# carlosluis/multiagent_planning

Measured on AMD Instinct MI355X. Metric: agent-QP solves/sec (K=15 horizon), higher is better.
Workload: dtype f64

## Files before the change

multiagent_planning_amd/csrc/dmpc_lists.hip:

```cpp

constexpr int NSEG = 3, SEG_STEPS = K / NSEG;
static_assert(NSEG * SEG_STEPS == K, "horizon segments");
template <typename TT>
__global__ void bbox_kernel(int total, int C, const TT *__restrict__ lT, float *__restrict__ bbox, float *__restrict__ bbox_nm )
{
    const int i = blockIdx.x * blockDim.x + threadIdx.x;
    if (i >= total) return;
    const int c = i % C;
    const size_t gs = (size_t)(i / C);
    const TT *src = lT + gs * N3 * C + c;
    float *dst = bbox + gs * (6 * NSEG) * C + c;
    for (int sg = 0; sg < NSEG; ++sg) {
        double lo[3] = {1e300, 1e300, 1e300}, hi[3] = {-1e300, -1e300, -1e300};
        for (int k = sg * SEG_STEPS; k < (sg + 1) * SEG_STEPS; ++k)
#pragma unroll
            for (int a = 0; a < 3; ++a) {
                const double v = (double)src[(size_t)(3 * k + a) * C];
                lo[a] = fmin(lo[a], v); hi[a] = fmax(hi[a], v);
            }
#pragma unroll
        for (int a = 0; a < 3; ++a) {
            const float flo = __double2float_rd(lo[a]), fhi = __double2float_ru(hi[a]);
            dst[(size_t)(6 * sg + 2 * a) * C] = flo; dst[(size_t)(6 * sg + 2 * a + 1) * C] = fhi;
            bbox_nm[(size_t)i * NBOX_NM + 6 * sg + 2 * a] = flo; bbox_nm[(size_t)i * NBOX_NM + 6 * sg + 2 * a + 1] = fhi;
        }
    }
}

template <typename TT>
__device__ __forceinline__ float nbrmajor_word(const TT *lT, int C, size_t t)
{
    const int l = (int)(t & 63), k4 = l >> 2, a4 = l & 3;
    const size_t gc = t >> 6, gs = gc / (size_t)C, c = gc - gs * (size_t)C;
    return (a4 < 3 && k4 < K) ? (float)lT[(gs * N3 + 3 * k4 + a4) * C + c] : 0.f;
}
template <typename TT>
__global__ void table_nbrmajor_kernel(size_t total, int C, const TT *__restrict__ lT, float *__restrict__ out, int *__restrict__ zbuf , size_t nz)
{
    const size_t t = (size_t)blockIdx.x * blockDim.x + threadIdx.x;
    for (size_t z = t; z < nz; z += (size_t)gridDim.x * blockDim.x) zbuf[z] = 0;
    if (t >= total) return;
    out[t] = nbrmajor_word(lT, C, t);
}

typedef float f4_t __attribute__((ext_vector_type(4)));
typedef const f4_t __attribute__((address_space(4))) *ConstF4;
__global__ __launch_bounds__(64) void nbr_kernel(int S, int G, int C, int g_local, int c_first, int c_count, int short_from, float R, float Rz,
                                                 const float *__restrict__ bbox, const float *__restrict__ bbox_nm, int cap, int *__restrict__ list,
                                                 int *__restrict__ cnt_out)
{
    constexpr int NB = 6 * NSEG;
    const int nblk = (c_count + 63) >> 6;
    const int part = blockIdx.x % NBR_PARTS, sb = blockIdx.x / NBR_PARTS;
    const int scene = sb / nblk, b = sb - scene * nblk;
    const int lane = threadIdx.x;
    const int ci = b * 64 + lane;
    const bool mine = ci < c_count;
    const int cl = c_first + (mine ? ci : 0);
    float ob[NB];
#pragma unroll
    for (int x = 0; x < NB; ++x) {
        const float v = bbox[((size_t)(g_local * S + scene) * NB + x) * C + cl];
        const float infl = (x % 6 < 4) ? R : Rz;
        ob[x] = (x & 1) ? v + infl : v - infl;
    }
    const int pcap = cap / NBR_PARTS;
    const size_t gid = (size_t)scene * c_count + (mine ? ci : 0);
    int *mylist = list + gid * (size_t)cap + (size_t)part * pcap;
    const long E = (long)G * C;
    const int e_lo = (int)(E * part / NBR_PARTS), e_hi = (int)(E * (part + 1) / NBR_PARTS);
    int cnt = 0;
    for (int e = e_lo; e < e_hi;) {
        const int r = e / C, j_lo = e - r * C;
        const int j_hi = (e_hi - e) < (C - j_lo) ? j_lo + (e_hi - e) : C;
        const int j_end = j_hi < C - ((short_from && r >= short_from) ? 1 : 0) ? j_hi : C - ((short_from && r >= short_from) ? 1 : 0);
        const float *base = bbox_nm + ((size_t)(r * S + scene) * C) * NBOX_NM;
        const int self = (r == g_local) ? cl : -1;
        for (int jc = j_lo; jc < j_end; ++jc) {
            const ConstF4 nb = (ConstF4)(unsigned long long)(base + (size_t)jc * NBOX_NM);
            const f4_t n0 = nb[0], n1 = nb[1], n2 = nb[2], n3 = nb[3], n4 = nb[4];
            const float nv[20] = {n0.x, n0.y, n0.z, n0.w, n1.x, n1.y, n1.z, n1.w, n2.x, n2.y, n2.z, n2.w, n3.x, n3.y, n3.z, n3.w, n4.x, n4.y, n4.z, n4.w};
            float sgm[NSEG];
#pragma unroll
            for (int sg = 0; sg < NSEG; ++sg) {
                const float a0 = nv[6 * sg] - ob[6 * sg + 1], a1 = ob[6 * sg] - nv[6 * sg + 1], a2 = nv[6 * sg + 2] - ob[6 * sg + 3];
                const float a3 = ob[6 * sg + 2] - nv[6 * sg + 3], a4 = nv[6 * sg + 4] - ob[6 * sg + 5], a5 = ob[6 * sg + 4] - nv[6 * sg + 5];
                sgm[sg] = fmaxf(__builtin_fmaxf(__builtin_fmaxf(a0, a1), a2), __builtin_fmaxf(__builtin_fmaxf(a3, a4), a5));
            }
            const float worst = __builtin_fminf(__builtin_fminf(sgm[0], sgm[1]), sgm[2]);
            if (worst <= 0.f && mine && jc != self) {
                if (cnt < pcap) mylist[cnt] = (r << 20) | jc;
                cnt++;
            }
        }
        e += j_hi - j_lo;
    }
    if (mine) cnt_out[gid * NBR_PARTS + part] = cnt > pcap ? -1 : cnt;
}

struct GridGeom {
    float org[3], inv[3];
    int n[3];
};
__device__ __forceinline__ int grid_coord(const GridGeom &g, int a, float x)
{
    const float t = (x - g.org[a]) * g.inv[a];
    const int c = (int)floorf(t);
    return c < 0 ? 0 : (c >= g.n[a] ? g.n[a] - 1 : c);
}
__device__ __forceinline__ int box_cell(const GridGeom &gg, const float (&lo)[3], const float (&hi)[3], float (&half)[3])
{
    int cc[3];
#pragma unroll
    for (int a = 0; a < 3; ++a) {
        half[a] = 0.5f * (hi[a] - lo[a]) * 1.0001f + 1e-5f;
        cc[a] = grid_coord(gg, a, 0.5f * (lo[a] + hi[a]));
    }
    return (cc[2] * gg.n[1] + cc[1]) * gg.n[0] + cc[0];
}
__global__ void grid_bin_kernel(int total, int S, int C, int short_from, GridGeom gg, const float *__restrict__ bbox_nm, int *__restrict__ cellof,
                                int *__restrict__ cnt, int *__restrict__ maxhalf)
{
    const int i = blockIdx.x * blockDim.x + threadIdx.x;
    const bool in = i < total;
    const int ii = in ? i : total - 1;
    const int c = ii % C, rs = ii / C, scene = rs % S, r = rs / S;
    const bool valid = in && !(short_from && r >= short_from && c == C - 1);
    const float *b = bbox_nm + (size_t)ii * NBOX_NM;
    const int ncell = gg.n[0] * gg.n[1] * gg.n[2];
    const int sc0 = __builtin_amdgcn_readfirstlane(scene);
    const bool uni = __all(scene == sc0);
    {
        const int sg = (int)blockIdx.y;
        float lo[3], hi[3], half[3];
#pragma unroll
        for (int a = 0; a < 3; ++a) { lo[a] = b[6 * sg + 2 * a]; hi[a] = b[6 * sg + 2 * a + 1]; }
        const int cell = box_cell(gg, lo, hi, half);
#pragma unroll
        for (int a = 0; a < 3; ++a) {
            int hb = valid ? __float_as_int(half[a]) : 0;
            int *dst = maxhalf + ((size_t)scene * NSEG + sg) * 3 + a;
            if (uni) {
#pragma unroll
                for (int off = 32; off > 0; off >>= 1) { const int o = __shfl_xor(hb, off); hb = o > hb ? o : hb; }
                if ((threadIdx.x & 63) == 0 && hb > *(volatile int *)dst) atomicMax(dst, hb);
            } else if (valid && hb > *(volatile int *)dst) atomicMax(dst, hb);
        }
        if (in) cellof[(size_t)sg * total + i] = valid ? cell : -1;
        if (valid) atomicAdd(cnt + ((size_t)scene * NSEG + sg) * ncell + cell, 1);
    }
}
__global__ void grid_scan_kernel(int ncell, int *__restrict__ cnt, int *__restrict__ start)
{
    __shared__ int part[1024];
    int *f = cnt + (size_t)blockIdx.x * ncell, *st = start + (size_t)blockIdx.x * (ncell + 1);
    const int per = (ncell + 1023) / 1024, lo = threadIdx.x * per, hi = lo + per < ncell ? lo + per : ncell;
    int a = 0;
    for (int c = lo; c < hi; ++c) a += f[c];
    part[threadIdx.x] = a;
    __syncthreads();
    for (int d = 1; d < 1024; d <<= 1) {
        const int v = threadIdx.x >= d ? part[threadIdx.x - d] : 0;
        __syncthreads();
        part[threadIdx.x] += v;
        __syncthreads();
    }
    int run = part[threadIdx.x] - a;
    for (int c = lo; c < hi; ++c) { st[c] = run; run += f[c]; f[c] = 0; }
    if (threadIdx.x == 1023) st[ncell] = part[1023];
}
__device__ __forceinline__ void chord_record(const f4_t *row , float e1z, int code, f4_t &r0, f4_t &r1)
{
    f4_t v[SEG_STEPS];
#pragma unroll
    for (int u = 0; u < SEG_STEPS; ++u) { v[u] = row[u]; v[u].z *= e1z; }
    const f4_t a0 = v[0], a1 = v[SEG_STEPS - 1];
    float dev2 = 0.f;
#pragma unroll
    for (int u = 1; u < SEG_STEPS - 1; ++u) {
        const float t = (float)u / (float)(SEG_STEPS - 1);
        const float dx = v[u].x - (a0.x + t * (a1.x - a0.x)), dy = v[u].y - (a0.y + t * (a1.y - a0.y)), dz = v[u].z - (a0.z + t * (a1.z - a0.z));
        dev2 = fmaxf(dev2, dx * dx + dy * dy + dz * dz);
    }
    r0.x = __int_as_float(code); r0.y = a0.x; r0.z = a0.y; r0.w = a0.z;
    r1.x = a1.x - a0.x; r1.y = a1.y - a0.y; r1.z = a1.z - a0.z; r1.w = sqrtf(dev2) * 1.0001f + 1e-5f;
}
__global__ void grid_fill_kernel(int total, int S, int C, int ncell, float e1z, const int *__restrict__ cellof, int *__restrict__ cnt, const int *__restrict__ start,
                                 const float *__restrict__ lrow, f4_t *__restrict__ ent)
{
    const int i = blockIdx.x * blockDim.x + threadIdx.x;
    if (i >= total) return;
    const int c = i % C, rs = i / C, scene = rs % S, r = rs / S;
    const size_t nag = (size_t)total / S;
#pragma unroll
    for (int sg = 0; sg < NSEG; ++sg) {
        const int cell = cellof[(size_t)sg * total + i];
        if (cell < 0) return;
        const size_t ss = (size_t)scene * NSEG + sg;
        const int pos = atomicAdd(cnt + ss * ncell + cell, 1);
        f4_t r0, r1;
        chord_record((const f4_t *)lrow + (size_t)i * 16 + SEG_STEPS * sg, e1z, (r << 20) | c, r0, r1);
        const size_t ei = ss * nag + start[ss * (ncell + 1) + cell] + pos;
        ent[ei] = r0; ent[(size_t)S * NSEG * nag + ei] = r1;
    }
}
template <typename TT>
__global__ __launch_bounds__(256) void grid_prep_kernel(int total, int C, int short_from, GridGeom gg, int nbA, const TT *__restrict__ lT, float *__restrict__ bbox,
                                                        float *__restrict__ bbox_nm, float *__restrict__ lrow, int *__restrict__ cellof, int *__restrict__ posof,
                                                        int *__restrict__ cnt, int *__restrict__ maxhalf)
{
    if ((int)blockIdx.x >= nbA) {
        const size_t t = (size_t)((int)blockIdx.x - nbA) * 256 + threadIdx.x;
        if (t >= (size_t)total * 64) return;
        lrow[t] = nbrmajor_word(lT, C, t);
        return;
    }
    __shared__ int mh[NSEG * 3];
    if (threadIdx.x < NSEG * 3) mh[threadIdx.x] = 0;
    __syncthreads();
    const int i = (int)blockIdx.x * 256 + (int)threadIdx.x;
    if (i < total) {
        const int c = i % C, r = i / C;
        const bool valid = !(short_from && r >= short_from && c == C - 1);
        const TT *src = lT + (size_t)r * N3 * C + c;
        float *dst = bbox + (size_t)r * (6 * NSEG) * C + c;
        const int ncell = gg.n[0] * gg.n[1] * gg.n[2];
#pragma unroll
        for (int sg = 0; sg < NSEG; ++sg) {
            double lo[3] = {1e300, 1e300, 1e300}, hi[3] = {-1e300, -1e300, -1e300};
#pragma unroll
            for (int k = sg * SEG_STEPS; k < (sg + 1) * SEG_STEPS; ++k)
#pragma unroll
                for (int a = 0; a < 3; ++a) {
                    const double v = (double)src[(size_t)(3 * k + a) * C];
                    lo[a] = fmin(lo[a], v); hi[a] = fmax(hi[a], v);
                }
            float flo[3], fhi[3], half[3];
#pragma unroll
            for (int a = 0; a < 3; ++a) {
                flo[a] = __double2float_rd(lo[a]); fhi[a] = __double2float_ru(hi[a]);
                dst[(size_t)(6 * sg + 2 * a) * C] = flo[a]; dst[(size_t)(6 * sg + 2 * a + 1) * C] = fhi[a];
                bbox_nm[(size_t)i * NBOX_NM + 6 * sg + 2 * a] = flo[a]; bbox_nm[(size_t)i * NBOX_NM + 6 * sg + 2 * a + 1] = fhi[a];
            }
            const int cell = box_cell(gg, flo, fhi, half);
#pragma unroll
            for (int a = 0; a < 3; ++a)
                if (valid) atomicMax(&mh[3 * sg + a], __float_as_int(half[a]));
            cellof[(size_t)sg * total + i] = valid ? cell : -1;
            posof[(size_t)sg * total + i] = valid ? atomicAdd(cnt + (size_t)sg * ncell + cell, 1) : 0;
        }
    }
    __syncthreads();
    if (threadIdx.x < NSEG * 3) { const int v = mh[threadIdx.x]; if (v > *(volatile int *)(maxhalf + threadIdx.x)) atomicMax(maxhalf + threadIdx.x, v); }
}
__global__ __launch_bounds__(256) void grid_fill2_kernel(int total, int C, int ncell, float e1z, const int *__restrict__ cellof, const int *__restrict__ posof,
                                                         const int *__restrict__ cnt, int *__restrict__ start, const float *__restrict__ lrow, f4_t *__restrict__ ent)
{
    int *st = (int *)dmpc_smem;
    __shared__ int wtot[NSEG][4];
    const int t = (int)threadIdx.x, lane = t & 63, wave = t >> 6;
    const int chunk = ((ncell + 255) / 256) | 1;
    const int lo = t * chunk, hi = lo + chunk < ncell ? lo + chunk : ncell;
#pragma unroll 4
    for (int j = t; j < ncell; j += 256)
#pragma unroll
        for (int sg = 0; sg < NSEG; ++sg) st[sg * (ncell + 1) + j] = cnt[(size_t)sg * ncell + j];
    __syncthreads();
    int sum[NSEG], inc[NSEG];
#pragma unroll
    for (int sg = 0; sg < NSEG; ++sg) sum[sg] = 0;
    for (int j = lo; j < hi; ++j)
#pragma unroll
        for (int sg = 0; sg < NSEG; ++sg) sum[sg] += st[sg * (ncell + 1) + j];
#pragma unroll
    for (int sg = 0; sg < NSEG; ++sg) inc[sg] = sum[sg];
#pragma unroll
    for (int off = 1; off < 64; off <<= 1)
#pragma unroll
        for (int sg = 0; sg < NSEG; ++sg) { const int o = __shfl_up(inc[sg], off); if (lane >= off) inc[sg] += o; }
    if (lane == 63)
#pragma unroll
        for (int sg = 0; sg < NSEG; ++sg) wtot[sg][wave] = inc[sg];
    __syncthreads();
    int run[NSEG];
#pragma unroll
    for (int sg = 0; sg < NSEG; ++sg) {
        run[sg] = inc[sg] - sum[sg];
        for (int w = 0; w < wave; ++w) run[sg] += wtot[sg][w];
        if (t == 255) st[sg * (ncell + 1) + ncell] = wtot[sg][0] + wtot[sg][1] + wtot[sg][2] + wtot[sg][3];
    }
    for (int j = lo; j < hi; ++j)
#pragma unroll
        for (int sg = 0; sg < NSEG; ++sg) { int *c = st + sg * (ncell + 1) + j; const int n = *c; *c = run[sg]; run[sg] += n; }
    __syncthreads();
    {
        const int all = NSEG * (ncell + 1), slice = (all + (int)gridDim.x - 1) / (int)gridDim.x;
        const int j0 = (int)blockIdx.x * slice, j1 = j0 + slice < all ? j0 + slice : all;
        for (int j = j0 + t; j < j1; j += 256) start[j] = st[j];
    }
    const int i = (int)blockIdx.x * 256 + t;
    if (i >= total) return;
    const int code = ((i / C) << 20) | (i % C);
#pragma unroll
    for (int sg = 0; sg < NSEG; ++sg) {
        const int cell = cellof[(size_t)sg * total + i];
        if (cell < 0) return;
        const int pos = posof[(size_t)sg * total + i];
        f4_t r0, r1;
        chord_record((const f4_t *)lrow + (size_t)i * 16 + SEG_STEPS * sg, e1z, code, r0, r1);
        const size_t ei = (size_t)sg * total + st[sg * (ncell + 1) + cell] + pos;
        ent[ei] = r0; ent[(size_t)NSEG * total + ei] = r1;
    }
}
constexpr int GQ_WAVES = NSEG;
constexpr int GQ_STAGE = 128;
inline size_t grid_query_lds(int nagents, int close_cap = 0)
{
    return (((size_t)((nagents + 31) / 32) * 4 + GQ_WAVES * GQ_STAGE * 4 + 15) & ~(size_t)15) + 16 * 16 + (close_cap > 0 ? 16 + (size_t)close_cap * 8 : 0);
}
typedef float f2_t __attribute__((ext_vector_type(2)));
__global__ __launch_bounds__(64 * GQ_WAVES) void grid_query_kernel(int S, int G, int C, int g_local, int c_first, int c_count, GridGeom gg, float R, float Rz, float e1z, float thr2,
                                                                   const float *__restrict__ bbox_nm, const float *__restrict__ lrow, const int *__restrict__ start,
                                                                   const f4_t *__restrict__ ent, const int *__restrict__ maxhalf, int cap, int cell_order,
                                                                   int *__restrict__ list, int *__restrict__ cnt_out,
                                                                   float thr_close, int close_cap, int *__restrict__ close_list, int *__restrict__ close_cnt)
{
    const int wave = __builtin_amdgcn_readfirstlane((int)(threadIdx.x >> 6)), lane = (int)(threadIdx.x & 63);
    const int gid = (int)blockIdx.x;
    const int nag = G * C, nwords = (nag + 31) >> 5, ncell = gg.n[0] * gg.n[1] * gg.n[2];
    const int scene = gid / c_count;
    int ci = gid - scene * c_count;
    if (cell_order) ci = __builtin_amdgcn_readfirstlane(__float_as_int(ent[(size_t)scene * NSEG * nag + ci].x) & 0xfffff);
    const int cl = c_first + ci;
    const int oid = scene * c_count + ci;
    unsigned *bits = (unsigned *)dmpc_smem;
    int *stage = (int *)(dmpc_smem + (size_t)nwords * 4) + wave * GQ_STAGE;
    f4_t *ownrow = (f4_t *)(dmpc_smem + (((size_t)nwords * 4 + GQ_WAVES * GQ_STAGE * 4 + 15) & ~(size_t)15));
    int *ccnt = (int *)(ownrow + 16), *crec = ccnt + 4;
    for (int i = (int)threadIdx.x; i < nwords; i += 64 * GQ_WAVES) bits[i] = 0u;
    if (close_cap > 0 && threadIdx.x == 0) *ccnt = 0;
    const size_t self_i = (size_t)(g_local * S + scene) * C + cl;
    if (threadIdx.x < 16) ownrow[lane] = ((const f4_t *)lrow)[self_i * 16 + lane];
    const ConstF4 ob4 = (ConstF4)(unsigned long long)(bbox_nm + self_i * NBOX_NM);
    const f4_t o0 = ob4[0], o1 = ob4[1], o2 = ob4[2], o3 = ob4[3], o4 = ob4[4];
    const float obx[18] = {o0.x, o0.y, o0.z, o0.w, o1.x, o1.y, o1.z, o1.w, o2.x, o2.y, o2.z, o2.w, o3.x, o3.y, o3.z, o3.w, o4.x, o4.y};
    __syncthreads();
    const int self_code = (g_local << 20) | cl;
    {
        const int sg = wave;
        int c_lo[3], c_hi[3];
#pragma unroll
        for (int a = 0; a < 3; ++a) {
            const float lo = sg == 0 ? obx[2 * a] : (sg == 1 ? obx[6 + 2 * a] : obx[12 + 2 * a]);
            const float hi = sg == 0 ? obx[2 * a + 1] : (sg == 1 ? obx[6 + 2 * a + 1] : obx[12 + 2 * a + 1]);
            const float infl = a < 2 ? R : Rz;
            const float reach = infl + __int_as_float(maxhalf[((size_t)scene * NSEG + sg) * 3 + a]);
            c_lo[a] = grid_coord(gg, a, lo - reach); c_hi[a] = grid_coord(gg, a, hi + reach);
        }
        f4_t oa0 = ownrow[SEG_STEPS * sg], oa1 = ownrow[SEG_STEPS * sg + SEG_STEPS - 1];
        oa0.z *= e1z; oa1.z *= e1z;
        const float odx = oa1.x - oa0.x, ody = oa1.y - oa0.y, odz = oa1.z - oa0.z;
        float odev2 = 0.f;
#pragma unroll
        for (int u = 1; u < SEG_STEPS - 1; ++u) {
            const f4_t o = ownrow[SEG_STEPS * sg + u];
            const float t = (float)u / (float)(SEG_STEPS - 1);
            const float dx = o.x - (oa0.x + t * odx), dy = o.y - (oa0.y + t * ody), dz = o.z * e1z - (oa0.z + t * odz);
            odev2 = fmaxf(odev2, dx * dx + dy * dy + dz * dz);
        }
        const float lim0 = sqrtf(thr2) + sqrtf(odev2) * 1.0001f + 2e-4f;
        const size_t ss = (size_t)scene * NSEG + sg;
        const int *st = start + ss * (ncell + 1);
        const f4_t *en = ent + ss * nag, *en2 = ent + (size_t)S * NSEG * nag + ss * nag;
        int nst = 0;
        auto traj_test = [&](int n) {
            const bool have = lane < n;
            const int code = stage[have ? lane : 0];
            const int r = code >> 20, jc = code & 0xfffff;
            const f4_t *row = (const f4_t *)lrow + ((size_t)(r * S + scene) * C + jc) * 16 + SEG_STEPS * sg;
            bool pass = false;
            int cmask = 0;
#pragma unroll 1
            for (int u = 0; u < SEG_STEPS; ++u) {
                const f4_t o = ownrow[SEG_STEPS * sg + u], w = row[u];
                const float dx = o.x - w.x, dy = o.y - w.y, dz = (o.z - w.z) * e1z;
                const float d2 = dx * dx + dy * dy + dz * dz;
                pass = pass || (d2 < thr2);
                cmask |= (d2 < thr_close) ? (1 << u) : 0;
            }
            if (have && pass) {
                const int idx = r * C + jc;
                atomicOr(bits + (idx >> 5), 1u << (idx & 31));
                if (cmask != 0) {
                    int pos = atomicAdd(ccnt, __popc(cmask));
                    while (cmask) {
                        const int u = __ffs(cmask) - 1;
                        cmask &= cmask - 1;
                        if (pos < close_cap) { crec[2 * pos] = code; crec[2 * pos + 1] = SEG_STEPS * sg + u; }
                        ++pos;
                    }
                }
            }
        };
        const int ny = c_hi[1] - c_lo[1] + 1, nruns_all = ny * (c_hi[2] - c_lo[2] + 1);
        const UDiv div_ny((unsigned)ny);
        for (int run0 = 0; run0 < nruns_all; run0 += 64) {
            const int nruns = nruns_all - run0 < 64 ? nruns_all - run0 : 64;
            int rb = 0, re = 0;
            if (lane < nruns) {
                int qz, qy;
                div_ny.divmod((unsigned)(run0 + lane), qz, qy);
                const int row0 = ((c_lo[2] + qz) * gg.n[1] + c_lo[1] + qy) * gg.n[0];
                rb = st[row0 + c_lo[0]]; re = st[row0 + c_hi[0] + 1];
            }
            const int len = re - rb;
            int pre = len;
            for (int off = 1; off < 64; off <<= 1) { const int o = __shfl_up(pre, off); if (lane >= off) pre += o; }
            const int tot = __builtin_amdgcn_readlane(pre, 63);
            const int basev = rb - (pre - len);
            const int nround = (tot + 63) >> 6;
            struct Rec { f4_t a, b; bool hv; };
            auto fetch = [&](int k, Rec &rc) {
                const int vi = 64 * k + lane;
                rc.hv = vi < tot;
                const int vq = rc.hv ? vi : tot - 1;
                int j = 0;
#pragma unroll
                for (int step = 32; step > 0; step >>= 1) { const int pm = __shfl(pre, j + step - 1); if (pm <= vq) j += step; }
                const size_t ei = (size_t)(__shfl(basev, j) + vq);
                rc.a = en[ei]; rc.b = en2[ei];
            };
            auto test = [&](const Rec &rc) {
                const float qx = rc.a.y - oa0.x, qy = rc.a.z - oa0.y, qz = rc.a.w - oa0.z;
                const float ex = rc.b.x - odx, ey = rc.b.y - ody, ez = rc.b.z - odz;
                const float ee = ex * ex + ey * ey + ez * ez, qe = qx * ex + qy * ey + qz * ez, qq = qx * qx + qy * qy + qz * qz;
                const float tt = __builtin_fminf(__builtin_fmaxf(-qe * __builtin_amdgcn_rcpf(__builtin_fmaxf(ee, 1e-20f)), 0.f), 1.f);
                const float d2 = qq + tt * (qe + qe + tt * ee);
                const float lim = lim0 + rc.b.w;
                const int c0 = __float_as_int(rc.a.x);
                const bool surv = rc.hv && c0 != self_code && d2 <= lim * lim;
                const unsigned long long m = __ballot(surv);
                if (m) {
                    if (surv) stage[nst + lanes_below(m, lane)] = c0;
                    nst += __popcll(m);
                    LSYNC();
                    if (nst >= 64) {
                        traj_test(64);
                        LSYNC();
                        const int keep = lane < nst - 64 ? stage[64 + lane] : 0;
                        LSYNC();
                        if (lane < nst - 64) stage[lane] = keep;
                        nst -= 64;
                        LSYNC();
                    }
                }
            };
            if (nround > 0) {
                Rec ra, rb2;
                fetch(0, ra);
                for (int k = 0; k < nround; k += 2) {
                    fetch(k + 1 < nround ? k + 1 : nround - 1, rb2);
                    test(ra);
                    if (k + 1 >= nround) break;
                    fetch(k + 2 < nround ? k + 2 : nround - 1, ra);
                    test(rb2);
                }
            }
        }
        if (nst > 0) traj_test(nst);
    }
    __syncthreads();
    if (wave == 1 && close_cap > 0) {
        const int n = *ccnt;
        int *dst = close_list + (size_t)oid * 2 * close_cap;
        if (n <= close_cap) for (int i = lane; i < 2 * n; i += 64) dst[i] = crec[i];
        if (lane == 0) close_cnt[oid] = n > close_cap ? -1 : n;
    }
    if (wave != 0) return;
    int *out = list + (size_t)oid * cap;
    int total = 0;
    const UDiv div_c((unsigned)C);
    for (int w0 = 0; w0 < nwords; w0 += 64) {
        unsigned word = w0 + lane < nwords ? bits[w0 + lane] : 0u;
        const int mycnt = __popc(word);
        int pre = mycnt;
        for (int off = 1; off < 64; off <<= 1) { const int o = __shfl_up(pre, off); if (lane >= off) pre += o; }
        const int wave_total = __builtin_amdgcn_readlane(pre, 63);
        int pos = total + pre - mycnt;
        while (word) {
            const int b = __ffs((int)word) - 1;
            word &= word - 1u;
            const int idx = ((w0 + lane) << 5) + b;
            int r = 0, jc = idx;
            if (G > 1) div_c.divmod((unsigned)idx, r, jc);
            if (pos < cap) out[pos] = (r << 20) | jc;
            ++pos;
        }
        total += wave_total;
    }
    if (lane == 0) cnt_out[(size_t)oid * NBR_PARTS] = total > cap ? -1 : total;
}
```

Baseline: 15.99 million.

## Map candidate slots to grid runs via LDS bitmap windows and DPP scans

Replaces the per-fetch 6-step shuffle binary search, which finds which cell run each candidate slot belongs to, with a per-wave LDS bitmap of run endpoints. Each fetch resolves its run index with mbcnt over that bitmap and reads the run base from LDS. Prefix sums now use DPP row operations instead of shfl_up loops, and the output-compaction loop skips all-zero word groups. The cost is more LDS per wave, extra LDS barriers and atomics for each 2048-slot window, and reliance on specific DPP control encodings being correct for a 64-lane wave.

Result: faster. 16.31 million (median of 6 runs) (+2.0%).

```diff
diff --git a/multiagent_planning_amd/csrc/dmpc_lists.hip b/multiagent_planning_amd/csrc/dmpc_lists.hip
--- a/multiagent_planning_amd/csrc/dmpc_lists.hip
+++ b/multiagent_planning_amd/csrc/dmpc_lists.hip
@@ -314,11 +314,25 @@
 }
 constexpr int GQ_WAVES = NSEG;
 constexpr int GQ_STAGE = 128;
+constexpr int GQ_RUNS = 64;
+constexpr int GQ_WIN = 2048;
+constexpr int GQ_WAVE_INTS = GQ_STAGE + GQ_RUNS + GQ_WIN / 32;
+static_assert(GQ_WIN / 32 == 64, "the window is one word per lane");
 inline size_t grid_query_lds(int nagents, int close_cap = 0)
 {
-    return (((size_t)((nagents + 31) / 32) * 4 + GQ_WAVES * GQ_STAGE * 4 + 15) & ~(size_t)15) + 16 * 16 + (close_cap > 0 ? 16 + (size_t)close_cap * 8 : 0);
+    return (((size_t)((nagents + 31) / 32) * 4 + GQ_WAVES * GQ_WAVE_INTS * 4 + 15) & ~(size_t)15) + 16 * 16 + (close_cap > 0 ? 16 + (size_t)close_cap * 8 : 0);
 }
 typedef float f2_t __attribute__((ext_vector_type(2)));
+__device__ __forceinline__ int wave_scan_add(int v)
+{
+    v += __builtin_amdgcn_update_dpp(0, v, 0x111, 0xf, 0xf, false);
+    v += __builtin_amdgcn_update_dpp(0, v, 0x112, 0xf, 0xf, false);
+    v += __builtin_amdgcn_update_dpp(0, v, 0x114, 0xf, 0xf, false);
+    v += __builtin_amdgcn_update_dpp(0, v, 0x118, 0xf, 0xf, false);
+    v += __builtin_amdgcn_update_dpp(0, v, 0x142, 0xa, 0xf, false);
+    v += __builtin_amdgcn_update_dpp(0, v, 0x143, 0xc, 0xf, false);
+    return v;
+}
 __global__ __launch_bounds__(64 * GQ_WAVES) void grid_query_kernel(int S, int G, int C, int g_local, int c_first, int c_count, GridGeom gg, float R, float Rz, float e1z, float thr2,
                                                                    const float *__restrict__ bbox_nm, const float *__restrict__ lrow, const int *__restrict__ start,
                                                                    const f4_t *__restrict__ ent, const int *__restrict__ maxhalf, int cap, int cell_order,
@@ -334,8 +348,10 @@
     const int cl = c_first + ci;
     const int oid = scene * c_count + ci;
     unsigned *bits = (unsigned *)dmpc_smem;
-    int *stage = (int *)(dmpc_smem + (size_t)nwords * 4) + wave * GQ_STAGE;
-    f4_t *ownrow = (f4_t *)(dmpc_smem + (((size_t)nwords * 4 + GQ_WAVES * GQ_STAGE * 4 + 15) & ~(size_t)15));
+    int *stage = (int *)(dmpc_smem + (size_t)nwords * 4) + wave * GQ_WAVE_INTS;
+    int *runbase = stage + GQ_STAGE;
+    unsigned *win = (unsigned *)(runbase + GQ_RUNS);
+    f4_t *ownrow = (f4_t *)(dmpc_smem + (((size_t)nwords * 4 + GQ_WAVES * GQ_WAVE_INTS * 4 + 15) & ~(size_t)15));
     int *ccnt = (int *)(ownrow + 16), *crec = ccnt + 4;
     for (int i = (int)threadIdx.x; i < nwords; i += 64 * GQ_WAVES) bits[i] = 0u;
     if (close_cap > 0 && threadIdx.x == 0) *ccnt = 0;
@@ -414,22 +430,14 @@
                 rb = st[row0 + c_lo[0]]; re = st[row0 + c_hi[0] + 1];
             }
             const int len = re - rb;
-            int pre = len;
-            for (int off = 1; off < 64; off <<= 1) { const int o = __shfl_up(pre, off); if (lane >= off) pre += o; }
+            const int pre = wave_scan_add(len);
             const int tot = __builtin_amdgcn_readlane(pre, 63);
-            const int basev = rb - (pre - len);
-            const int nround = (tot + 63) >> 6;
+            const unsigned long long ne = __ballot(len > 0);
+            LSYNC();
+            if (len > 0) runbase[lanes_below(ne, lane)] = rb - (pre - len);
+            const int endpos = (len > 0 && pre < tot) ? pre - 1 : -1;
+            int ord0 = 0;
             struct Rec { f4_t a, b; bool hv; };
-            auto fetch = [&](int k, Rec &rc) {
-                const int vi = 64 * k + lane;
-                rc.hv = vi < tot;
-                const int vq = rc.hv ? vi : tot - 1;
-                int j = 0;
-#pragma unroll
-                for (int step = 32; step > 0; step >>= 1) { const int pm = __shfl(pre, j + step - 1); if (pm <= vq) j += step; }
-                const size_t ei = (size_t)(__shfl(basev, j) + vq);
-                rc.a = en[ei]; rc.b = en2[ei];
-            };
             auto test = [&](const Rec &rc) {
                 const float qx = rc.a.y - oa0.x, qy = rc.a.z - oa0.y, qz = rc.a.w - oa0.z;
                 const float ex = rc.b.x - odx, ey = rc.b.y - ody, ez = rc.b.z - odz;
@@ -455,15 +463,35 @@
                     }
                 }
             };
-            if (nround > 0) {
-                Rec ra, rb2;
-                fetch(0, ra);
-                for (int k = 0; k < nround; k += 2) {
-                    fetch(k + 1 < nround ? k + 1 : nround - 1, rb2);
-                    test(ra);
-                    if (k + 1 >= nround) break;
-                    fetch(k + 2 < nround ? k + 2 : nround - 1, ra);
-                    test(rb2);
+            for (int w0 = 0; w0 < tot; w0 += GQ_WIN) {
+                win[lane] = 0u;
+                LSYNC();
+                if ((unsigned)(endpos - w0) < (unsigned)GQ_WIN) atomicOr(win + ((endpos - w0) >> 5), 1u << ((endpos - w0) & 31));
+                LSYNC();
+                const unsigned myw = win[lane];
+                const int cumi = wave_scan_add(__popc(myw));
+                const int cumw = ord0 + cumi - __popc(myw);
+                ord0 += __builtin_amdgcn_readlane(cumi, 63);
+                const int nround = ((tot - w0 < GQ_WIN ? tot - w0 : GQ_WIN) + 63) >> 6;
+                auto fetch = [&](int k, Rec &rc) {
+                    const int vi = w0 + 64 * k + lane;
+                    rc.hv = vi < tot;
+                    const int vq = rc.hv ? vi : tot - 1;
+                    const unsigned mlo = (unsigned)__builtin_amdgcn_readlane((int)myw, 2 * k), mhi = (unsigned)__builtin_amdgcn_readlane((int)myw, 2 * k + 1);
+                    const int o = (int)__builtin_amdgcn_mbcnt_hi(mhi, __builtin_amdgcn_mbcnt_lo(mlo, (unsigned)__builtin_amdgcn_readlane(cumw, 2 * k)));
+                    const unsigned eb = (unsigned)(runbase[o] + vq) << 4;
+                    rc.a = *(const f4_t *)((const char *)en + eb); rc.b = *(const f4_t *)((const char *)en2 + eb);
+                };
+                if (nround > 0) {
+                    Rec ra, rb2;
+                    fetch(0, ra);
+                    for (int k = 0; k < nround; k += 2) {
+                        fetch(k + 1 < nround ? k + 1 : nround - 1, rb2);
+                        test(ra);
+                        if (k + 1 >= nround) break;
+                        fetch(k + 2 < nround ? k + 2 : nround - 1, ra);
+                        test(rb2);
+                    }
                 }
             }
         }
@@ -482,9 +510,9 @@
     const UDiv div_c((unsigned)C);
     for (int w0 = 0; w0 < nwords; w0 += 64) {
         unsigned word = w0 + lane < nwords ? bits[w0 + lane] : 0u;
+        if (__ballot(word != 0u) == 0ull) continue;
         const int mycnt = __popc(word);
-        int pre = mycnt;
-        for (int off = 1; off < 64; off <<= 1) { const int o = __shfl_up(pre, off); if (lane >= off) pre += o; }
+        const int pre = wave_scan_add(mycnt);
         const int wave_total = __builtin_amdgcn_readlane(pre, 63);
         int pos = total + pre - mycnt;
         while (word) {
```
